# mwickert/scikit-dsp-comm

Hardware: AMD Instinct MI355X
Metric: complex64 MSamples/s (FIR-1024 tap, 2^26 samples) (higher is better)
Workload: dtype c64

## Files before the change

scikit-dsp-comm_amd/csrc/fir_ols.hip:

```cpp
#include "skdsp_internal.hpp"
#include "ols_tables.hpp"
#include <cstdlib>
#include <cstdio>


namespace skdsp {

using namespace ols;
typedef float v4f_t __attribute__((ext_vector_type(4)));

struct OlsPlan {
    int ntaps = 0;
    int ov = 0;
    int V = 0;
    float4 *T1 = nullptr, *T2 = nullptr, *Hp = nullptr;
};

struct OlsArgs {
    const cf *x;
    cf *y;
    int64_t n, n_hist;
    const float4 *T1, *T2, *Hp;
    int ov, V, a0;
    int keep;
// ... 285 lines not shown
__device__ __forceinline__ void load_tile_xr(const OlsArgs &A, int64_t tile, int t, cf *v)
{
    const float *xr = reinterpret_cast<const float *>(A.x);
    const int64_t in0 = tile * A.V - A.ov;
    const bool interior = A.aligned && in0 >= -A.n_hist && in0 + kN <= A.n;
    int tt = t;
    asm volatile("" : "+v"(tt));
    if (interior) {
#pragma unroll
        for (int a = 0; a < 16; ++a) {
            const v2f_t r = __builtin_nontemporal_load(reinterpret_cast<const v2f_t *>(xr + in0) + (unsigned)(a * 256 + tt));
            v[2 * a] = make_float2(r.x, 0.f);
            v[2 * a + 1] = make_float2(r.y, 0.f);
        }
    } else {
#pragma unroll
        for (int a = 0; a < 16; ++a) {
#pragma unroll
            for (int e = 0; e < 2; ++e) {
                const int64_t g = in0 + 512 * a + 2 * tt + e;
                v[2 * a + e] = make_float2((g >= -A.n_hist && g < A.n) ? xr[g] : 0.f, 0.f);
            }
        }
    }
}

template <bool REAL, bool XR = false> __device__ __forceinline__ void load_any(const OlsArgs &A, int64_t tile, int t, cf *v)
{
    if (XR) load_tile_xr(A, tile, t, v); else if (REAL) load_tile_real(A, tile, t, v); else load_tile(A, tile, t, v);
}
template <bool REAL, bool DEC> __device__ __forceinline__ void store_any(const OlsArgs &A, int64_t tile, int t, const cf *v, float4 *lds)
{
    if (REAL) store_tile_real<DEC>(A, tile, t, v, lds); else store_tile<DEC>(A, tile, t, v, lds);
}

__device__ __forceinline__ void lanes_swap_halves(float &e0, float &e1)
{
    const auto r = __builtin_amdgcn_permlane32_swap(__float_as_uint(e0), __float_as_uint(e1), false, false);
    e0 = __uint_as_float(r[0]);
    e1 = __uint_as_float(r[1]);
}
__device__ __forceinline__ int up_lane_pos(int t)
{
    const int lane = t & 63;
    return 128 * (t >> 6) + (lane < 32 ? 2 * lane : 2 * (lane - 32) + 1);
}

template <bool DEC> __device__ __forceinline__ void store_tile_up(const OlsArgs &A, int64_t tile, int ph, int t, const cf *v)
{
    int a0 = A.a0;
    asm volatile("" : "+s"(a0));
    int tt = t;
    asm volatile("" : "+v"(tt));
    const int pos = up_lane_pos(tt);
    const int64_t out0 = tile * A.V;
    char *ub = reinterpret_cast<char *>(A.y) + out0 * A.up_sb + A.up_pb0 + (int64_t)ph * A.up_pbs;
    const int64_t left = A.n - out0;
    const int lim = (left > (1 << 20) ? (1 << 20) : (int)left) - pos;
    const bool whole = left >= A.V;
    const unsigned b0 = (unsigned)pos * (unsigned)A.up_sb, b1 = b0 + 64u * (unsigned)A.up_sb;
    const size_t step = (size_t)512 * A.up_sb;
    const unsigned M = (unsigned)A.dec;
    const int64_t jt = out0 * A.up + ph, q0 = DEC ? jt / A.dec : 0;
    const unsigned r0 = DEC ? (unsigned)(jt - q0 * A.dec) : 0u;
    const int64_t qleft = A.n_keep - q0;
    const int qlim = qleft > (1 << 24) ? (1 << 24) : (int)qleft;
    cf *yq = A.y + q0;
#pragma unroll
    for (int a = 0; a < 16; ++a) {
        if (a < a0) continue;
        cf e0 = v[2 * a], e1 = v[2 * a + 1];
        lanes_swap_halves(e0.x, e1.x);
        lanes_swap_halves(e0.y, e1.y);
        const int i = 512 * (a - a0);
        if (DEC) {
            const unsigned j0 = r0 + (unsigned)(i + pos) * (unsigned)A.up, j1 = j0 + 64u * (unsigned)A.up;
            const unsigned k0 = (unsigned)(((unsigned long long)j0 * A.dec_magic) >> 32), k1 = (unsigned)(((unsigned long long)j1 * A.dec_magic) >> 32);
            if (k0 * M == j0 && (int)k0 < qlim && (whole || i < lim)) yq[k0] = e0;
            if (k1 * M == j1 && (int)k1 < qlim && (whole || i + 64 < lim)) yq[k1] = e1;
            continue;
        }
        char *ua = ub + (size_t)(a - a0) * step;
        if (whole || i < lim) *reinterpret_cast<cf *>(ua + b0) = e0;
        if (whole || i + 64 < lim) *reinterpret_cast<cf *>(ua + b1) = e1;
    }
}

template <bool DEC> __device__ __forceinline__ void store_tile_real_up(const OlsArgs &A, int64_t pair, int ph, int t, const cf *v)
{
    int a0 = A.a0;
    asm volatile("" : "+s"(a0));
    int tt = t;
    asm volatile("" : "+v"(tt));
    const int pos = up_lane_pos(tt);
    const int64_t outA = (2 * pair) * A.V;
    char *ua0 = reinterpret_cast<char *>(A.y) + outA * A.up_sb + A.up_pb0 + (int64_t)ph * A.up_pbs;
    char *ub0 = ua0 + (size_t)A.V * A.up_sb;
    const int64_t left = A.n - outA;
    const int lim = (left > (1 << 20) ? (1 << 20) : (int)left) - pos;
    const int limb = lim - A.V;
    const bool whole = left >= 2 * (int64_t)A.V;
    const unsigned b0 = (unsigned)pos * (unsigned)A.up_sb, b1 = b0 + 64u * (unsigned)A.up_sb;
    const size_t step = (size_t)512 * A.up_sb;
    const unsigned M = (unsigned)A.dec;
    const int64_t jt = outA * A.up + ph, q0 = DEC ? jt / A.dec : 0;
    const unsigned r0 = DEC ? (unsigned)(jt - q0 * A.dec) : 0u;
    const int64_t qleft = A.n_keep - q0;
    const int qlim = qleft > (1 << 24) ? (1 << 24) : (int)qleft;
    float *yq = reinterpret_cast<float *>(A.y) + q0;
    const unsigned jv = (unsigned)A.V * (unsigned)A.up;
#pragma unroll
    for (int a = 0; a < 16; ++a) {
        if (a < a0) continue;
        cf e0 = v[2 * a], e1 = v[2 * a + 1];
        lanes_swap_halves(e0.x, e1.x);
        lanes_swap_halves(e0.y, e1.y);
        const int i = 512 * (a - a0);
        if (DEC) {
            const unsigned j0 = r0 + (unsigned)(i + pos) * (unsigned)A.up, j1 = j0 + 64u * (unsigned)A.up;
            auto keep = [&](unsigned j, float val, bool inside) __attribute__((always_inline)) {
                const unsigned k = (unsigned)(((unsigned long long)j * A.dec_magic) >> 32);
                if (k * M == j && (int)k < qlim && inside) yq[k] = val;
            };
            keep(j0, e0.x, whole || i < lim);
            keep(j1, e1.x, whole || i + 64 < lim);
            keep(j0 + jv, e0.y, whole || i < limb);
            keep(j1 + jv, e1.y, whole || i + 64 < limb);
            continue;
        }
        char *ua = ua0 + (size_t)(a - a0) * step, *ub = ub0 + (size_t)(a - a0) * step;
        if (whole || i < lim) *reinterpret_cast<float *>(ua + b0) = e0.x;
        if (whole || i + 64 < lim) *reinterpret_cast<float *>(ua + b1) = e1.x;
        if (whole || i < limb) *reinterpret_cast<float *>(ub + b0) = e0.y;
        if (whole || i + 64 < limb) *reinterpret_cast<float *>(ub + b1) = e1.y;
    }
}


__device__ __forceinline__ OlsCareful ols_careful_args(const OlsArgs &A, int ph, bool cx)
{
    OlsCareful c;
    c.x = A.x; c.y = A.y; c.n = A.n; c.n_hist = A.n_hist; c.n_keep = A.n_keep; c.up_pitch = A.up_pitch;
    c.V = A.V; c.dec = A.dec; c.up = A.up;
    const int esz = cx ? 8 : 4;
    c.L = A.up_sb / esz;
    c.p0 = (A.up_pb0 + ph * A.up_pbs) / esz;
    c.cf = A.cf;
    return c;
}

template <bool REAL, bool DEC, bool UP = false, bool XR = false>
__global__ __launch_bounds__(256, 2) void ols_tile_kernel(OlsArgs A)
{
    __shared__ float4 lds[kLdsUnits + 2 * kT2Units];
    __shared__ unsigned long long ols_noted;
    if (threadIdx.x == 0) ols_noted = 0;
    constexpr int HS = (DEC && !UP) ? (REAL ? 4 : 5) : 0;
    float4 *T2f = lds + kLdsUnits;
    float4 *T2t = lds + kLdsUnits + kT2Units;
    const int t = threadIdx.x;

    {
        const float4 w = A.T2[t];
        T2f[t] = w;
        T2t[(t & 15) * 16 + (t >> 4)] = w;
    }
    cf tw[16];
#pragma unroll
    for (int k1 = 1; k1 < 16; ++k1) tw[k1] = lo(A.T1[k1 * 256 + t]);
    tw[0] = make_float2(1.f, 0.f);

    __syncthreads();
    int it = 0;
    float4 hh[16];
    int64_t tile = (gridDim.x % 8 == 0) ? (int64_t)(blockIdx.x % 8) * (gridDim.x / 8) + blockIdx.x / 8
                                                                 : (int64_t)blockIdx.x;
    const bool t0_last = A.halo_flag != nullptr;
    auto phys = [&](int64_t w) -> int64_t {
        if (UP) return (int64_t)((unsigned)w / (unsigned)A.up);
        return t0_last ? (w + 1 < A.ntiles ? w + 1 : 0) : w;
    };
    auto phase_of = [&](int64_t w) -> int { return (int)((unsigned)w % (unsigned)A.up); };
    if (!UP) load_H(t, A.Hp, hh);
    cf v[32];
    if (tile < A.ntiles) {
        if (t0_last && phys(tile) == 0) wait_halo(A);
        load_any<REAL, XR>(A, phys(tile), t, v);
    }
    if constexpr (XR) {
#pragma unroll
        for (int i = 0; i < 32; i += 8)
            asm volatile("" ::"v"(v[i].x), "v"(v[i + 1].x), "v"(v[i + 2].x), "v"(v[i + 3].x), "v"(v[i + 4].x), "v"(v[i + 5].x), "v"(v[i + 6].x), "v"(v[i + 7].x));
    } else {
#pragma unroll
    for (int i = 0; i < 32; i += 8)
        asm volatile("" ::"v"(v[i].x), "v"(v[i].y), "v"(v[i + 1].x), "v"(v[i + 1].y), "v"(v[i + 2].x), "v"(v[i + 2].y),
                     "v"(v[i + 3].x), "v"(v[i + 3].y), "v"(v[i + 4].x), "v"(v[i + 4].y), "v"(v[i + 5].x), "v"(v[i + 5].y),
                     "v"(v[i + 6].x), "v"(v[i + 6].y), "v"(v[i + 7].x), "v"(v[i + 7].y));
    }
    for (; tile < A.ntiles; tile += gridDim.x, ++it) {
        if (HS > 0) {
            int tt = t;
            asm volatile("" : "+v"(tt));
#pragma unroll
            for (int j = 16 - HS; j < 16; ++j) hh[j] = vld(reinterpret_cast<const volatile float4 *>(A.Hp) + (unsigned)(j * 256 + tt));
        }
        if (UP) {
            int tt = t;
            asm volatile("" : "+v"(tt));
            const volatile float4 *hp = reinterpret_cast<const volatile float4 *>(A.Hp) + (size_t)phase_of(tile) * 4096;
#pragma unroll
            for (int j = 0; j < 16; ++j) hh[j] = vld(hp + (unsigned)(j * 256 + tt));
        }
        if (REAL) fwd_pass1_real(t, v, tw, lds); else fwd_pass1(t, v, tw, lds);
        __syncthreads();
        cf Z[32];
        fwd_pass23(t, T2f, lds, Z);
        mul_H(hh, Z);
        const int64_t next = tile + gridDim.x;
        cf nx[32];
        __builtin_amdgcn_s_setprio(3);
        if (next < A.ntiles) {
            if (t0_last && phys(next) == 0) wait_halo(A);
            load_any<REAL, XR>(A, phys(next), t, nx);
        }
        __builtin_amdgcn_s_setprio(0);
        inv_pass32(t, T2t, lds, Z);
        __syncthreads();
        inv_pass1(t, tw, lds, v);
        if constexpr (XR) {
#pragma unroll
            for (int i = 0; i < 32; i += 8)
                asm volatile("" ::"v"(nx[i].x), "v"(nx[i + 1].x), "v"(nx[i + 2].x), "v"(nx[i + 3].x), "v"(nx[i + 4].x), "v"(nx[i + 5].x), "v"(nx[i + 6].x), "v"(nx[i + 7].x)
                             : "memory");
        } else {
#pragma unroll
        for (int i = 0; i < 32; i += 8)
            asm volatile("" ::"v"(nx[i].x), "v"(nx[i].y), "v"(nx[i + 1].x), "v"(nx[i + 1].y), "v"(nx[i + 2].x), "v"(nx[i + 2].y),
                         "v"(nx[i + 3].x), "v"(nx[i + 3].y), "v"(nx[i + 4].x), "v"(nx[i + 4].y), "v"(nx[i + 5].x), "v"(nx[i + 5].y),
                         "v"(nx[i + 6].x), "v"(nx[i + 6].y), "v"(nx[i + 7].x), "v"(nx[i + 7].y)
                         : "memory");
        }
        __builtin_amdgcn_s_setprio(3);
        if (UP) {
            if (!DEC && A.up_pitch) {
                OlsArgs B = A;
                B.y = REAL ? reinterpret_cast<cf *>(reinterpret_cast<float *>(A.y) + (int64_t)phase_of(tile) * A.up_pitch) : A.y + (int64_t)phase_of(tile) * A.up_pitch;
                store_any<REAL, false>(B, phys(tile), t, v, lds);
            } else if (REAL) {
                store_tile_real_up<DEC>(A, phys(tile), phase_of(tile), t, v);
            } else {
                store_tile_up<DEC>(A, phys(tile), phase_of(tile), t, v);
            }
        } else {
            store_any<REAL, DEC>(A, phys(tile), t, v, lds);
        }
        __builtin_amdgcn_s_setprio(0);
        if (__builtin_expect(__any(not_finite(v[31].x) | not_finite(v[31].y)), 0)) careful_note(&ols_noted, it);
#pragma unroll
        for (int i = 0; i < 32; ++i) v[i] = nx[i];
#ifdef SK_OLS_KEEP_B3
        __syncthreads();
#else
        if constexpr (REAL || DEC || UP || XR) __syncthreads();
#endif
    }
    const unsigned long long noted = careful_noted(&ols_noted);
    if (__builtin_expect(noted != 0, 0)) {
        int64_t w = (gridDim.x % 8 == 0) ? (int64_t)(blockIdx.x % 8) * (gridDim.x / 8) + blockIdx.x / 8 : (int64_t)blockIdx.x;
        for (int64_t k = 0; w < A.ntiles; w += gridDim.x, ++k)
            if (careful_step_noted(noted, k))
                careful_ols_tile<float, REAL, DEC, UP, XR>(ols_careful_args(A, UP ? phase_of(w) : 0, !(REAL || XR)), phys(w), UP ? phase_of(w) : 0, t);
    }
}


template <bool REAL, int MF>
__global__ __launch_bounds__(256, 2) void ols_fold_kernel(OlsArgs A)
{
    __shared__ float4 lds[kLdsUnits + 2 * kT2Units];
    __shared__ unsigned long long ols_noted;
    if (threadIdx.x == 0) ols_noted = 0;
    float4 *T2f = lds + kLdsUnits, *T2t = lds + kLdsUnits + kT2Units;
    const int t = threadIdx.x;
    {
        const float4 w = A.T2[t];
        T2f[t] = w;
        T2t[(t & 15) * 16 + (t >> 4)] = w;
    }
    cf tw[16];
#pragma unroll
    for (int k1 = 1; k1 < 16; ++k1) tw[k1] = lo(A.T1[k1 * 256 + t]);
    tw[0] = make_float2(1.f, 0.f);
    __syncthreads();
    float4 hh[16];
    auto first_tile = [&]() -> int64_t { return (gridDim.x % 8 == 0) ? (int64_t)(blockIdx.x % 8) * (gridDim.x / 8) + blockIdx.x / 8 : (int64_t)blockIdx.x; };
    int64_t tile = first_tile();
    load_H(t, A.Hp, hh);
    cf v[32];
    if (tile < A.ntiles) load_any<REAL, false>(A, tile, t, v);
#pragma unroll
    for (int i = 0; i < 32; i += 8)
        asm volatile("" ::"v"(v[i].x), "v"(v[i].y), "v"(v[i + 1].x), "v"(v[i + 1].y), "v"(v[i + 2].x), "v"(v[i + 2].y),
                     "v"(v[i + 3].x), "v"(v[i + 3].y), "v"(v[i + 4].x), "v"(v[i + 4].y), "v"(v[i + 5].x), "v"(v[i + 5].y),
                     "v"(v[i + 6].x), "v"(v[i + 6].y), "v"(v[i + 7].x), "v"(v[i + 7].y));
    constexpr int LS = MF / 2;
    const int b = t >> 4, q = t & 15;
    const bool active = q % LS == 0;
    const int j0 = (32 / MF) * b + q / LS;
    constexpr int JA = 512 / MF;
    for (int64_t step = 0; tile < A.ntiles; tile += gridDim.x, ++step) {
        if (REAL) fwd_pass1_real(t, v, tw, lds); else fwd_pass1(t, v, tw, lds);
        __syncthreads();
        cf Z[32];
        fwd_pass23(t, T2f, lds, Z);
        mul_H(hh, Z);
        const int64_t next = tile + gridDim.x;
        cf nx[32];
        __builtin_amdgcn_s_setprio(3);
        if (next < A.ntiles) load_any<REAL, false>(A, next, t, nx);
        __builtin_amdgcn_s_setprio(0);
        inv_pass32_fold<MF>(t, T2t, lds, Z);
        __syncthreads();
        cf o[16];
#pragma unroll
        for (int a = 0; a < 16; ++a) o[a] = make_float2(0.f, 0.f);
        inv_pass1_fold<MF>(t, tw, lds, o);
#pragma unroll
        for (int i = 0; i < 32; i += 8)
            asm volatile("" ::"v"(nx[i].x), "v"(nx[i].y), "v"(nx[i + 1].x), "v"(nx[i + 1].y), "v"(nx[i + 2].x), "v"(nx[i + 2].y),
                         "v"(nx[i + 3].x), "v"(nx[i + 3].y), "v"(nx[i + 4].x), "v"(nx[i + 4].y), "v"(nx[i + 5].x), "v"(nx[i + 5].y),
                         "v"(nx[i + 6].x), "v"(nx[i + 6].y), "v"(nx[i + 7].x), "v"(nx[i + 7].y)
                         : "memory");
        __builtin_amdgcn_s_setprio(3);
        if (active) {
            int a0 = A.a0;
            asm volatile("" : "+s"(a0));
            const int Mr = A.dec / MF;
            const int64_t n_out = A.n_keep / A.dec;
            const int VD = A.V / MF;
            const int64_t e0 = (REAL ? 2 * tile : tile) * (int64_t)VD;
            const int64_t q0 = Mr > 1 ? e0 / Mr : e0;
            const unsigned r0 = Mr > 1 ? (unsigned)(e0 - q0 * Mr) : 0u;
            auto put = [&](unsigned el, auto val, auto *yp) __attribute__((always_inline)) {
                if (Mr > 1) {
                    const unsigned g = r0 + el;
                    const unsigned k = (unsigned)(((unsigned long long)g * A.dec_magic) >> 32);
                    if (k * (unsigned)Mr == g && q0 + k < n_out) __builtin_nontemporal_store(val, yp + (q0 + k));
                } else if (q0 + el < n_out) {
                    __builtin_nontemporal_store(val, yp + (q0 + el));
                }
            };
#pragma unroll
            for (int a = 0; a < 16; ++a) {
                if (a < a0) continue;
                const unsigned el = (unsigned)(j0 + JA * (a - a0));
                if (REAL) {
                    put(el, o[a].x, reinterpret_cast<float *>(A.y));
                    put(el + (unsigned)VD, o[a].y, reinterpret_cast<float *>(A.y));
                } else {
                    put(el, v2f_t{o[a].x, o[a].y}, reinterpret_cast<v2f_t *>(A.y));
                }
            }
        }
        __builtin_amdgcn_s_setprio(0);
        if (__builtin_expect(__any(active && (not_finite(o[15].x) | not_finite(o[15].y))), 0)) careful_note(&ols_noted, step);
#pragma unroll
        for (int i = 0; i < 32; ++i) v[i] = nx[i];
#ifdef SK_OLS_KEEP_B3
        __syncthreads();
#else
        if constexpr (REAL) __syncthreads();
#endif
    }
    const unsigned long long noted = careful_noted(&ols_noted);
    if (__builtin_expect(noted != 0, 0)) {
        int64_t w = first_tile();
        for (int64_t k = 0; w < A.ntiles; w += gridDim.x, ++k)
            if (careful_step_noted(noted, k)) careful_ols_tile<float, REAL, true, false, false>(ols_careful_args(A, 0, !REAL), w, 0, t);
    }
}


template <bool REAL, int LF>
__device__ __forceinline__ void load_rep(const OlsArgs &A, int64_t tile, int t, cf *in)
{
    constexpr int LS = LF / 2, JA = 512 / LF;
    const int b = t >> 4, q = t & 15;
#pragma unroll
    for (int a = 0; a < 16; ++a) in[a] = make_float2(0.f, 0.f);
    if (q % LS != 0) return;
    const int j0 = (32 / LF) * b + q / LS;
    const int Lr = A.rep_lr;
    const int64_t in0 = (REAL ? 2 * tile : tile) * (int64_t)A.V - A.ov;
    const int64_t e0 = in0 / LF;
    int64_t q0 = e0, r0 = 0;
    if (Lr > 1) {
        q0 = e0 / Lr;
        r0 = e0 - q0 * Lr;
        if (r0 < 0) { r0 += Lr; q0 -= 1; }
    }
    const int VD = A.V / LF;
    auto fetch = [&](unsigned d, int64_t &idx) -> bool {
        if (Lr == 1) { idx = q0 + d; return true; }
        const unsigned g = (unsigned)r0 + d;
        const unsigned k = (unsigned)(((unsigned long long)g * A.rep_magic) >> 32);
        idx = q0 + k;
        return k * (unsigned)Lr == g;
    };
    const bool interior = Lr == 1 && A.aligned && e0 >= -A.rep_hist && e0 + kN / LF + (REAL ? VD : 0) <= A.n_in;
    int tt = j0;
    asm volatile("" : "+v"(tt));
    if (interior) {
        if (REAL) {
            const float *xa = reinterpret_cast<const float *>(A.x) + e0, *xb = xa + VD;
#pragma unroll
            for (int a = 0; a < 16; ++a) in[a] = make_float2(__builtin_nontemporal_load(xa + (unsigned)(JA * a + tt)), __builtin_nontemporal_load(xb + (unsigned)(JA * a + tt)));
        } else {
            const v2f_t *xc = reinterpret_cast<const v2f_t *>(A.x) + e0;
#pragma unroll
            for (int a = 0; a < 16; ++a) {
                const v2f_t r = __builtin_nontemporal_load(xc + (unsigned)(JA * a + tt));
                in[a] = make_float2(r.x, r.y);
            }
        }
        return;
    }
#pragma unroll
    for (int a = 0; a < 16; ++a) {
        int64_t ia, ib;
        if (REAL) {
            const float *xr = reinterpret_cast<const float *>(A.x);
            float va = 0.f, vb = 0.f;
            if (fetch((unsigned)(JA * a + tt), ia) && ia >= -A.rep_hist && ia < A.n_in) va = xr[ia];
            if (fetch((unsigned)(JA * a + tt + VD), ib) && ib >= -A.rep_hist && ib < A.n_in) vb = xr[ib];
            in[a] = make_float2(va, vb);
        } else if (fetch((unsigned)(JA * a + tt), ia) && ia >= -A.rep_hist && ia < A.n_in) {
            in[a] = A.x[ia];
        }
    }
}

template <bool REAL, int LF>
__global__ __launch_bounds__(256, 2) void ols_rep_kernel(OlsArgs A)
{
    __shared__ float4 lds[kLdsUnits + 2 * kT2Units];
    __shared__ unsigned long long ols_noted;
    if (threadIdx.x == 0) ols_noted = 0;
    float4 *T2f = lds + kLdsUnits, *T2t = lds + kLdsUnits + kT2Units;
    const int t = threadIdx.x;
    {
        const float4 w = A.T2[t];
        T2f[t] = w;
        T2t[(t & 15) * 16 + (t >> 4)] = w;
    }
    cf tw[16];
#pragma unroll
    for (int k1 = 1; k1 < 16; ++k1) tw[k1] = lo(A.T1[k1 * 256 + t]);
    tw[0] = make_float2(1.f, 0.f);
    __syncthreads();
    float4 hh[16];
    auto first_tile = [&]() -> int64_t { return (gridDim.x % 8 == 0) ? (int64_t)(blockIdx.x % 8) * (gridDim.x / 8) + blockIdx.x / 8 : (int64_t)blockIdx.x; };
    int64_t tile = first_tile();
    load_H(t, A.Hp, hh);
    cf in[16];
    if (tile < A.ntiles) load_rep<REAL, LF>(A, tile, t, in);
#pragma unroll
    for (int i = 0; i < 16; i += 8)
        asm volatile("" ::"v"(in[i].x), "v"(in[i].y), "v"(in[i + 1].x), "v"(in[i + 1].y), "v"(in[i + 2].x), "v"(in[i + 2].y),
                     "v"(in[i + 3].x), "v"(in[i + 3].y), "v"(in[i + 4].x), "v"(in[i + 4].y), "v"(in[i + 5].x), "v"(in[i + 5].y),
                     "v"(in[i + 6].x), "v"(in[i + 6].y), "v"(in[i + 7].x), "v"(in[i + 7].y));
    for (int64_t step = 0; tile < A.ntiles; tile += gridDim.x, ++step) {
        fwd_pass1_rep<LF>(t, in, tw, lds);
        __syncthreads();
        cf Z[32];
        fwd_pass23_rep<LF>(t, T2f, lds, Z);
        mul_H(hh, Z);
        const int64_t next = tile + gridDim.x;
        cf nx[16];
        __builtin_amdgcn_s_setprio(3);
        if (next < A.ntiles) load_rep<REAL, LF>(A, next, t, nx);
        __builtin_amdgcn_s_setprio(0);
        inv_pass32(t, T2t, lds, Z);
        __syncthreads();
        cf v[32];
        inv_pass1(t, tw, lds, v);
#pragma unroll
        for (int i = 0; i < 16; i += 8)
            asm volatile("" ::"v"(nx[i].x), "v"(nx[i].y), "v"(nx[i + 1].x), "v"(nx[i + 1].y), "v"(nx[i + 2].x), "v"(nx[i + 2].y),
                         "v"(nx[i + 3].x), "v"(nx[i + 3].y), "v"(nx[i + 4].x), "v"(nx[i + 4].y), "v"(nx[i + 5].x), "v"(nx[i + 5].y),
                         "v"(nx[i + 6].x), "v"(nx[i + 6].y), "v"(nx[i + 7].x), "v"(nx[i + 7].y)
                         : "memory");
        __builtin_amdgcn_s_setprio(3);
        store_any<REAL, false>(A, tile, t, v, lds);
        __builtin_amdgcn_s_setprio(0);
        if (__builtin_expect(__any(not_finite(v[31].x) | not_finite(v[31].y)), 0)) careful_note(&ols_noted, step);
#pragma unroll
        for (int i = 0; i < 16; ++i) in[i] = nx[i];
        __syncthreads();
    }
    const unsigned long long noted = careful_noted(&ols_noted);
    if (__builtin_expect(noted != 0, 0)) {
        int64_t w = first_tile();
        for (int64_t k = 0; w < A.ntiles; w += gridDim.x, ++k)
            if (careful_step_noted(noted, k))
                careful_fir_range<float, !REAL>(A.x, A.y, A.rep_hist, A.n, (REAL ? 2 * w : w) * (int64_t)A.V, (REAL ? 2 : 1) * (int64_t)A.V, A.rep_L, 1, A.cf, t);
    }
}

bool fir_ols_supported(const FirHandle *h)
{
    if (h->ntaps < 2 || h->ntaps - 1 > 4096) return false;
    return h->dtype == SKDSP_C64 || (h->dtype == SKDSP_F32 && !h->taps_complex);
}

static int build_plan(const FirHandle *h, int up, OlsPlan **out, int kind = 0)
{
    if (kind == 1) {
        const int T = (h->ntaps + up - 1) / up;
        OlsPlan *p = new OlsPlan();
        p->ntaps = T;
        p->ov = ((T - 1 + 511) / 512) * 512;
        if (p->ov == 0) p->ov = 512;
        p->V = kN - p->ov;
        std::vector<float4> T1, T2, Hp, Hall;
        make_T1(T1);
        make_T2(T2);
        std::vector<double> ph((size_t)T * 2);
        for (int k = 0; k < up / 2; ++k) {
            std::fill(ph.begin(), ph.end(), 0.0);
            for (int t = 0; t < T; ++t)
                for (int c = 0; c < 2; ++c) {
                    const int j = 2 * k + c + up * t;
                    if (j < h->ntaps) ph[(size_t)2 * t + c] = (double)up * h->taps_host[j];
                }
            make_Hp(ph.data(), T, 2, Hp);
            Hall.insert(Hall.end(), Hp.begin(), Hp.end());
        }
        hipError_t e;
        if ((e = hipMalloc((void **)&p->T1, T1.size() * sizeof(float4))) != hipSuccess ||
            (e = hipMalloc((void **)&p->T2, T2.size() * sizeof(float4))) != hipSuccess ||
            (e = hipMalloc((void **)&p->Hp, Hall.size() * sizeof(float4))) != hipSuccess ||
            (e = hipMemcpy(p->T1, T1.data(), T1.size() * sizeof(float4), hipMemcpyHostToDevice)) != hipSuccess ||
            (e = hipMemcpy(p->T2, T2.data(), T2.size() * sizeof(float4), hipMemcpyHostToDevice)) != hipSuccess ||
            (e = hipMemcpy(p->Hp, Hall.data(), Hall.size() * sizeof(float4), hipMemcpyHostToDevice)) != hipSuccess) {
            fir_ols_free(p);
            return hip_fail(e, "ols tables (paired phases)", __FILE__, __LINE__);
        }
        *out = p;
        return SKDSP_OK;
    }
    const int comp = h->taps_complex ? 2 : 1;
    const int T = kind == 3 ? h->ntaps : (h->ntaps + up - 1) / up;
    const int q_first = kind == 2 ? up - 1 : 0;
    OlsPlan *p = new OlsPlan();
    p->ntaps = T;
    p->ov = ((T - 1 + 511) / 512) * 512;
    if (p->ov == 0) p->ov = 512;
    p->V = kN - p->ov;
    std::vector<float4> T1, T2, Hp, Hall;
    make_T1(T1);
    make_T2(T2);
    if (up == 1) {
        make_Hp(h->taps_host.data(), h->ntaps, comp, Hall);
    } else if (kind == 3) {
        std::vector<double> scaled(h->taps_host);
        for (double &v : scaled) v *= (double)up;
        make_Hp(scaled.data(), h->ntaps, comp, Hall);
    } else {
        std::vector<double> ph((size_t)T * comp);
        for (int q = q_first; q < up; ++q) {
            std::fill(ph.begin(), ph.end(), 0.0);
            for (int t = 0; t < T; ++t) {
                const int k = q + up * t;
                if (k >= h->ntaps) break;
                for (int c = 0; c < comp; ++c) ph[(size_t)t * comp + c] = (double)up * h->taps_host[(size_t)k * comp + c];
            }
            make_Hp(ph.data(), T, comp, Hp);
            Hall.insert(Hall.end(), Hp.begin(), Hp.end());
        }
    }
    hipError_t e;
    if ((e = hipMalloc((void **)&p->T1, T1.size() * sizeof(float4))) != hipSuccess ||
        (e = hipMalloc((void **)&p->T2, T2.size() * sizeof(float4))) != hipSuccess ||
        (e = hipMalloc((void **)&p->Hp, Hall.size() * sizeof(float4))) != hipSuccess) {
        fir_ols_free(p);
        return hip_fail(e, "hipMalloc(ols tables)", __FILE__, __LINE__);
    }
    if ((e = hipMemcpy(p->T1, T1.data(), T1.size() * sizeof(float4), hipMemcpyHostToDevice)) != hipSuccess ||
        (e = hipMemcpy(p->T2, T2.data(), T2.size() * sizeof(float4), hipMemcpyHostToDevice)) != hipSuccess ||
        (e = hipMemcpy(p->Hp, Hall.data(), Hall.size() * sizeof(float4), hipMemcpyHostToDevice)) != hipSuccess) {
        fir_ols_free(p);
        return hip_fail(e, "hipMemcpy(ols tables)", __FILE__, __LINE__);
    }
    *out = p;
    return SKDSP_OK;
}

static int ensure_plan(FirHandle *h)
{
    if (h->ols) return SKDSP_OK;
    return build_plan(h, 1, &h->ols);
// ... 241 lines not shown
```

scikit-dsp-comm_amd/csrc/ols_core.hpp:

```cpp
#pragma once

#include <type_traits>
#if defined(__HIPCC__)
#include <hip/hip_runtime.h>
#define SK_HD __host__ __device__ __forceinline__
#define SK_UNROLL _Pragma("unroll")
#else
#include <cmath>
#define SK_UNROLL
struct float2 { float x, y; };
struct float4 { float x, y, z, w; };
static inline float2 make_float2(float x, float y) { return float2{x, y}; }
static inline float4 make_float4(float x, float y, float z, float w) { return float4{x, y, z, w}; }
#define SK_HD inline
#endif

namespace skdsp {
namespace ols {

typedef float2 cf;

constexpr int kN = 8192;
constexpr int kThreads = 256;
constexpr int kRowPitch = 272;
constexpr int kLdsUnits = 16 * kRowPitch;
constexpr int kT2Units = 256;

#define SK_C32                                                                                             \
    {1.0f, 0.98078528040323043f, 0.92387953251128674f, 0.83146961230254524f, 0.70710678118654757f,        \
     0.55557023301960229f, 0.38268343236508984f, 0.19509032201612833f, 0.0f, -0.19509032201612819f,       \
     -0.38268343236508973f, -0.55557023301960196f, -0.70710678118654746f, -0.83146961230254535f,           \
     -0.92387953251128674f, -0.98078528040323043f, -1.0f, -0.98078528040323043f, -0.92387953251128685f,    \
     -0.83146961230254546f, -0.70710678118654768f, -0.55557023301960218f, -0.38268343236509034f,           \
     -0.19509032201612866f, 0.0f, 0.19509032201612828f, 0.38268343236509f, 0.55557023301960184f,           \
     0.70710678118654735f, 0.83146961230254524f, 0.92387953251128652f, 0.98078528040323032f}
#define SK_S32                                                                                             \
    {0.0f, 0.19509032201612825f, 0.38268343236508978f, 0.55557023301960218f, 0.70710678118654746f,         \
     0.83146961230254524f, 0.92387953251128674f, 0.98078528040323043f, 1.0f, 0.98078528040323043f,         \
     0.92387953251128674f, 0.83146961230254546f, 0.70710678118654757f, 0.55557023301960218f,               \
     0.38268343236508989f, 0.19509032201612861f, 0.0f, -0.19509032201612836f, -0.38268343236508967f,       \
     -0.55557023301960196f, -0.70710678118654746f, -0.83146961230254524f, -0.92387953251128652f,           \
     -0.98078528040323032f, -1.0f, -0.98078528040323043f, -0.92387953251128663f, -0.83146961230254546f,    \
     -0.70710678118654768f, -0.55557023301960218f, -0.38268343236509039f, -0.19509032201612872f}

#if defined(__HIP_DEVICE_COMPILE__)
typedef float v2f __attribute__((ext_vector_type(2)));
SK_HD v2f V(cf a) { v2f r; r.x = a.x; r.y = a.y; return r; }
SK_HD cf C(v2f a) { return make_float2(a.x, a.y); }
SK_HD cf cadd(cf a, cf b) { return C(V(a) + V(b)); }
SK_HD cf csub(cf a, cf b) { return C(V(a) - V(b)); }
SK_HD cf cmul(cf a, cf w)
{
    v2f r;
    asm("v_pk_mul_f32 %0, %1, %2 op_sel_hi:[1,0]\n\t"
        "v_pk_fma_f32 %0, %1, %2, %0 op_sel:[1,1,0] op_sel_hi:[0,1,1] neg_lo:[0,1,0]"
        : "=&v"(r) : "v"(V(a)), "v"(V(w)));
    return C(r);
}
SK_HD cf cmulc(cf a, cf w)
{
    v2f r;
    asm("v_pk_mul_f32 %0, %1, %2 op_sel_hi:[1,0]\n\t"
        "v_pk_fma_f32 %0, %1, %2, %0 op_sel:[1,1,0] op_sel_hi:[0,1,1] neg_hi:[0,1,0]"
        : "=&v"(r) : "v"(V(a)), "v"(V(w)));
    return C(r);
}
template <bool INV> SK_HD cf cmul_k(cf a, float c, float s)
{
    v2f K;
    K.x = c; K.y = s;
    v2f r;
    if (INV)
        asm("v_pk_mul_f32 %0, %1, %2 op_sel_hi:[1,0]\n\t"
            "v_pk_fma_f32 %0, %1, %2, %0 op_sel:[1,1,0] op_sel_hi:[0,1,1] neg_lo:[0,1,0]"
            : "=&v"(r) : "v"(V(a)), "s"(K));
    else
        asm("v_pk_mul_f32 %0, %1, %2 op_sel_hi:[1,0]\n\t"
            "v_pk_fma_f32 %0, %1, %2, %0 op_sel:[1,1,0] op_sel_hi:[0,1,1] neg_hi:[0,1,0]"
            : "=&v"(r) : "v"(V(a)), "s"(K));
    return C(r);
}
template <bool INV> SK_HD cf madd_mi(cf p, cf d)
{
    v2f r;
    if (INV) asm("v_pk_add_f32 %0, %1, %2 op_sel:[0,1] op_sel_hi:[1,0] neg_lo:[0,1]" : "=v"(r) : "v"(V(p)), "v"(V(d)));
    else asm("v_pk_add_f32 %0, %1, %2 op_sel:[0,1] op_sel_hi:[1,0] neg_hi:[0,1]" : "=v"(r) : "v"(V(p)), "v"(V(d)));
    return C(r);
}
SK_HD cf cneg(cf a) { return C(-V(a)); }
#else
SK_HD cf cadd(cf a, cf b) { return make_float2(a.x + b.x, a.y + b.y); }
SK_HD cf csub(cf a, cf b) { return make_float2(a.x - b.x, a.y - b.y); }
SK_HD cf cmul(cf a, cf b) { return make_float2(a.x * b.x - a.y * b.y, a.x * b.y + a.y * b.x); }
SK_HD cf cmulc(cf a, cf b) { return make_float2(a.x * b.x + a.y * b.y, a.y * b.x - a.x * b.y); }
template <bool INV> SK_HD cf cmul_k(cf a, float c, float s)
{
    return INV ? make_float2(a.x * c - a.y * s, a.y * c + a.x * s) : make_float2(a.x * c + a.y * s, a.y * c - a.x * s);
}
template <bool INV> SK_HD cf madd_mi(cf p, cf d)
{
    return INV ? make_float2(p.x - d.y, p.y + d.x) : make_float2(p.x + d.y, p.y - d.x);
}
SK_HD cf cneg(cf a) { return make_float2(-a.x, -a.y); }
#endif
#if defined(__HIP_DEVICE_COMPILE__)
struct cf2 { v2f re, im; };
SK_HD cf2 make_cf2(cf re_pair, cf im_pair) { return cf2{V(re_pair), V(im_pair)}; }
SK_HD cf2 cadd(cf2 a, cf2 b) { return cf2{a.re + b.re, a.im + b.im}; }
SK_HD cf2 csub(cf2 a, cf2 b) { return cf2{a.re - b.re, a.im - b.im}; }
SK_HD cf2 cneg(cf2 a) { return cf2{-a.re, -a.im}; }
template <bool INV> SK_HD cf2 madd_mi(cf2 p, cf2 d) { return INV ? cf2{p.re - d.im, p.im + d.re} : cf2{p.re + d.im, p.im - d.re}; }
template <bool INV> SK_HD cf2 cmul_k(cf2 a, float c, float s)
{
    return INV ? cf2{a.re * c - a.im * s, a.im * c + a.re * s} : cf2{a.re * c + a.im * s, a.im * c - a.re * s};
}
SK_HD cf column(cf2 a, int e) { return e ? make_float2(a.re.y, a.im.y) : make_float2(a.re.x, a.im.x); }
template <int COL> SK_HD cf soa_cmul(cf2 a, cf w)
{
    v2f r;
    if (COL == 0)
        asm("v_pk_mul_f32 %0, %1, %3 op_sel:[0,0] op_sel_hi:[0,1]\n\t"
            "v_pk_fma_f32 %0, %2, %3, %0 op_sel:[0,1,0] op_sel_hi:[0,0,1] neg_lo:[0,1,0]"
            : "=&v"(r) : "v"(a.re), "v"(a.im), "v"(V(w)));
    else
        asm("v_pk_mul_f32 %0, %1, %3 op_sel:[1,0] op_sel_hi:[1,1]\n\t"
            "v_pk_fma_f32 %0, %2, %3, %0 op_sel:[1,1,0] op_sel_hi:[1,0,1] neg_lo:[0,1,0]"
            : "=&v"(r) : "v"(a.re), "v"(a.im), "v"(V(w)));
    return C(r);
}
#else
struct cf2 { float re[2], im[2]; };
SK_HD cf2 make_cf2(cf re_pair, cf im_pair) { return cf2{{re_pair.x, re_pair.y}, {im_pair.x, im_pair.y}}; }
SK_HD cf2 cadd(cf2 a, cf2 b) { return cf2{{a.re[0] + b.re[0], a.re[1] + b.re[1]}, {a.im[0] + b.im[0], a.im[1] + b.im[1]}}; }
SK_HD cf2 csub(cf2 a, cf2 b) { return cf2{{a.re[0] - b.re[0], a.re[1] - b.re[1]}, {a.im[0] - b.im[0], a.im[1] - b.im[1]}}; }
SK_HD cf2 cneg(cf2 a) { return cf2{{-a.re[0], -a.re[1]}, {-a.im[0], -a.im[1]}}; }
SK_HD cf column(cf2 a, int e) { return make_float2(a.re[e], a.im[e]); }
SK_HD cf2 from_columns(cf c0, cf c1) { return cf2{{c0.x, c1.x}, {c0.y, c1.y}}; }
template <bool INV> SK_HD cf2 madd_mi(cf2 p, cf2 d) { return from_columns(madd_mi<INV>(column(p, 0), column(d, 0)), madd_mi<INV>(column(p, 1), column(d, 1))); }
template <bool INV> SK_HD cf2 cmul_k(cf2 a, float c, float s) { return from_columns(cmul_k<INV>(column(a, 0), c, s), cmul_k<INV>(column(a, 1), c, s)); }
template <int COL> SK_HD cf soa_cmul(cf2 a, cf w) { return cmul(column(a, COL), w); }
#endif

template <bool INV, class E> SK_HD E msub_mi(E p, E d) { return madd_mi<!INV>(p, d); }
template <bool INV> SK_HD cf mul_mi(cf a) { return madd_mi<INV>(make_float2(0.f, 0.f), a); }
template <bool INV> SK_HD cf2 mul_mi(cf2 a) { return madd_mi<INV>(make_cf2(make_float2(0.f, 0.f), make_float2(0.f, 0.f)), a); }

template <bool INV> SK_HD void dft4_ip(cf &x0, cf &x1, cf &x2, cf &x3)
{
    const cf s02 = cadd(x0, x2), d02 = csub(x0, x2), s13 = cadd(x1, x3), d13 = csub(x1, x3);
    x0 = cadd(s02, s13);
    x2 = csub(s02, s13);
    x1 = madd_mi<INV>(d02, d13);
    x3 = msub_mi<INV>(d02, d13);
}

template <int N, int K, bool INV, class E> SK_HD E twmul(E a)
{
    constexpr int k32 = ((K % N) * (32 / N)) & 31;
    constexpr float Ct[32] = SK_C32;
    constexpr float St[32] = SK_S32;
    if constexpr (k32 == 0) return a;
    else if constexpr (k32 == 8) return mul_mi<INV>(a);
    else if constexpr (k32 == 16) return cneg(a);
    else if constexpr (k32 == 24) return mul_mi<!INV>(a);
    else return cmul_k<INV>(a, Ct[k32], St[k32]);
}

template <int N, int K, bool INV, class T> SK_HD void bfly_tw(T E, T O, T &Xa, T &Xb)
{
    constexpr int k32 = ((K % N) * (32 / N)) & 31;
    if constexpr (k32 == 8) {
        Xa = madd_mi<INV>(E, O);
        Xb = msub_mi<INV>(E, O);
    } else if constexpr (k32 == 24) {
        Xa = msub_mi<INV>(E, O);
        Xb = madd_mi<INV>(E, O);
    } else {
        const T t = twmul<N, K, INV>(O);
        Xa = cadd(E, t);
        Xb = csub(E, t);
    }
}

template <int I, int E, class F> SK_HD void static_for(F &&f)
{
    if constexpr (I < E) {
        f(std::integral_constant<int, I>{});
        static_for<I + 1, E>(static_cast<F &&>(f));
    }
}

template <class T, int N, int S, bool INV> struct DftT {
    static SK_HD void run(const T *x, T *X)
    {
        if constexpr (N == 1) {
            X[0] = x[0];
        } else if constexpr (N == 2) {
            X[0] = cadd(x[0], x[S]);
            X[1] = csub(x[0], x[S]);
        } else if constexpr (N == 4) {
            const T s02 = cadd(x[0], x[2 * S]), d02 = csub(x[0], x[2 * S]);
            const T s13 = cadd(x[S], x[3 * S]), d13 = csub(x[S], x[3 * S]);
            X[0] = cadd(s02, s13);
            X[2] = csub(s02, s13);
            X[1] = madd_mi<INV>(d02, d13);
            X[3] = msub_mi<INV>(d02, d13);
        } else if constexpr (N == 8) {
            T E[4], O[4];
            DftT<T, 4, 2 * S, INV>::run(x, E);
            DftT<T, 4, 2 * S, INV>::run(x + S, O);
            static_for<0, 4>([&](auto kc) {
                constexpr int k = decltype(kc)::value;
                bfly_tw<8, k, INV>(E[k], O[k], X[k], X[k + 4]);
            });
        } else {
            constexpr int M = N / 4;
            T S0[M], S1[M], S2[M], S3[M];
            DftT<T, M, 4 * S, INV>::run(x, S0);
            DftT<T, M, 4 * S, INV>::run(x + S, S1);
            DftT<T, M, 4 * S, INV>::run(x + 2 * S, S2);
            DftT<T, M, 4 * S, INV>::run(x + 3 * S, S3);
            static_for<0, M>([&](auto kc) {
                constexpr int k = decltype(kc)::value;
                const T t0 = S0[k];
                const T t1 = twmul<N, k, INV>(S1[k]);
                const T t2 = twmul<N, 2 * k, INV>(S2[k]);
                const T t3 = twmul<N, 3 * k, INV>(S3[k]);
                const T s02 = cadd(t0, t2), d02 = csub(t0, t2);
                const T s13 = cadd(t1, t3), d13 = csub(t1, t3);
                X[k] = cadd(s02, s13);
                X[k + 2 * M] = csub(s02, s13);
                X[k + M] = madd_mi<INV>(d02, d13);
                X[k + 3 * M] = msub_mi<INV>(d02, d13);
            });
        }
    }
};
template <int N, int S, bool INV> using Dft = DftT<cf, N, S, INV>;

SK_HD int lds_unit(int row_k1, int mid, int q) { return row_k1 * kRowPitch + mid * 17 + q; }

SK_HD cf lo(float4 f) { return make_float2(f.x, f.y); }
SK_HD cf hi(float4 f) { return make_float2(f.z, f.w); }
SK_HD float4 pack(cf a, cf b) { return make_float4(a.x, a.y, b.x, b.y); }

template <int K, bool INV> SK_HD cf mul_w8192(cf a)
{
    constexpr float C[16] = {1.0f, 0.99999970586288223f, 0.99999882345170188f, 0.99999735276697821f, 0.99999529380957619f, 0.99999264658070719f, 0.9999894110819284f, 0.9999855873151432f, 0.99998117528260111f, 0.99997617498689761f, 0.99997058643097414f, 0.99996440961811828f, 0.9999576445519639f, 0.99995029123649048f, 0.99994234967602391f, 0.999933819875236f};
    constexpr float S[16] = {0.0f, 0.00076699031874270449f, 0.0015339801862847655f, 0.002300969151425805f, 0.0030679567629659761f, 0.0038349425697062275f, 0.0046019261204485705f, 0.0053689069639963425f, 0.0061358846491544753f, 0.0069028587247297558f, 0.007669828739531097f, 0.0084367942423697988f, 0.0092037547820598194f, 0.0099707099074180308f, 0.010737659167264491f, 0.011504602110422714f};
    if constexpr (K == 0) return a;
    else if constexpr (INV) return make_float2(a.x * C[K] - a.y * S[K], a.y * C[K] + a.x * S[K]);
    else return make_float2(a.x * C[K] + a.y * S[K], a.y * C[K] - a.x * S[K]);
}

SK_HD void fwd_pass1(int t, const cf *v, const cf *tw, float4 *lds)
{
    cf in[16], o0[16], o1[16];
    SK_UNROLL
    for (int a = 0; a < 16; ++a) in[a] = v[2 * a];
    Dft<16, 1, false>::run(in, o0);
    SK_UNROLL
    for (int a = 0; a < 16; ++a) in[a] = v[2 * a + 1];
    Dft<16, 1, false>::run(in, o1);
    const int b = t >> 4, q = t & 15;
    lds[lds_unit(0, b, q)] = pack(o0[0], o1[0]);
    static_for<1, 16>([&](auto kc) {
        constexpr int k1 = decltype(kc)::value;
        lds[lds_unit(k1, b, q)] = pack(cmul(o0[k1], tw[k1]), cmul(mul_w8192<k1, false>(o1[k1]), tw[k1]));
    });
}

SK_HD void fwd_pass1_real(int t, const cf *v, const cf *tw, float4 *lds)
{
    cf2 in[16], o[16];
    SK_UNROLL
    for (int a = 0; a < 16; ++a) in[a] = make_cf2(v[2 * a], v[2 * a + 1]);
    DftT<cf2, 16, 1, false>::run(in, o);
    const int b = t >> 4, q = t & 15;
    lds[lds_unit(0, b, q)] = pack(column(o[0], 0), column(o[0], 1));
    static_for<1, 16>([&](auto kc) {
        constexpr int k1 = decltype(kc)::value;
        lds[lds_unit(k1, b, q)] = pack(soa_cmul<0>(o[k1], tw[k1]), mul_w8192<k1, false>(soa_cmul<1>(o[k1], tw[k1])));
    });
}

SK_HD void fwd_pass23(int t, const float4 *T2 , float4 *lds, cf *Z)
{
    const int k1 = t >> 4, q = t & 15;
    cf in0[16], in1[16], o0[16], o1[16];
    SK_UNROLL
    for (int b = 0; b < 16; ++b) {
        const float4 f = lds[lds_unit(k1, b, q)];
        in0[b] = lo(f);
        in1[b] = hi(f);
    }
    Dft<16, 1, false>::run(in0, o0);
    Dft<16, 1, false>::run(in1, o1);
    lds[lds_unit(k1, 0, q)] = pack(o0[0], o1[0]);
    SK_UNROLL
    for (int k2 = 1; k2 < 16; ++k2) {
        const float4 w = T2[k2 * 16 + q];
        lds[lds_unit(k1, k2, q)] = pack(cmul(o0[k2], lo(w)), cmul(o1[k2], hi(w)));
    }
    const int k2 = q;
    cf z[32];
    SK_UNROLL
    for (int qq = 0; qq < 16; ++qq) {
        const float4 f = lds[lds_unit(k1, k2, qq)];
        z[2 * qq] = lo(f);
        z[2 * qq + 1] = hi(f);
    }
    Dft<32, 1, false>::run(z, Z);
}

SK_HD void load_H(int t, const float4 *Hp, float4 *hh)
{
    SK_UNROLL
    for (int j = 0; j < 16; ++j) hh[j] = Hp[j * 256 + t];
}
SK_HD void mul_H(const float4 *hh, cf *Z)
{
    SK_UNROLL
    for (int j = 0; j < 16; ++j) {
        Z[2 * j] = cmul(Z[2 * j], lo(hh[j]));
        Z[2 * j + 1] = cmul(Z[2 * j + 1], hi(hh[j]));
    }
}

SK_HD void inv_pass32(int t, const float4 *T2t , float4 *lds, const cf *Z)
{
    const int k1 = t >> 4, k2 = t & 15;
    cf z[32];
    Dft<32, 1, true>::run(Z, z);
    SK_UNROLL
    for (int qq = 0; qq < 16; ++qq) {
        const float4 w = T2t[qq * 16 + k2];
        lds[lds_unit(k1, k2, qq)] = pack(cmulc(z[2 * qq], lo(w)), cmulc(z[2 * qq + 1], hi(w)));
    }
    const int q = k2;
    cf in0[16], in1[16], o0[16], o1[16];
    SK_UNROLL
    for (int kk = 0; kk < 16; ++kk) {
        const float4 f = lds[lds_unit(k1, kk, q)];
        in0[kk] = lo(f);
        in1[kk] = hi(f);
    }
    Dft<16, 1, true>::run(in0, o0);
    Dft<16, 1, true>::run(in1, o1);
    SK_UNROLL
    for (int b = 0; b < 16; ++b) lds[lds_unit(k1, b, q)] = pack(o0[b], o1[b]);
}

SK_HD void inv_pass1(int t, const cf *tw, const float4 *lds, cf *v)
{
    const int b = t >> 4, q = t & 15;
    cf in0[16], in1[16], o0[16], o1[16];
    {
        const float4 f = lds[lds_unit(0, b, q)];
        in0[0] = lo(f);
        in1[0] = hi(f);
    }
    static_for<1, 16>([&](auto kc) {
        constexpr int k1 = decltype(kc)::value;
        const float4 f = lds[lds_unit(k1, b, q)];
        in0[k1] = cmulc(lo(f), tw[k1]);
        in1[k1] = mul_w8192<k1, true>(cmulc(hi(f), tw[k1]));
    });
    Dft<16, 1, true>::run(in0, o0);
    Dft<16, 1, true>::run(in1, o1);
    SK_UNROLL
    for (int a = 0; a < 16; ++a) {
        v[2 * a] = o0[a];
        v[2 * a + 1] = o1[a];
    }
}

template <int MF> SK_HD void inv_pass32_fold(int t, const float4 *T2t , float4 *lds, const cf *Z)
{
    constexpr int R = 32 / MF, LS = MF / 2;
    const int k1 = t >> 4, k2 = t & 15;
    cf F[R], z[R];
    SK_UNROLL
    for (int k = 0; k < R; ++k) {
        cf acc = Z[k];
        SK_UNROLL
        for (int m = 1; m < MF; ++m) acc = cadd(acc, Z[k + R * m]);
        F[k] = acc;
    }
    Dft<R, 1, true>::run(F, z);
    cf *l2 = reinterpret_cast<cf *>(lds);
    SK_UNROLL
    for (int cp = 0; cp < R; ++cp) {
        const int qq = cp * LS;
        l2[2 * lds_unit(k1, k2, qq)] = cmulc(z[cp], lo(T2t[qq * 16 + k2]));
    }
    const int q = k2;
    if (q % LS == 0) {
        cf in0[16], o0[16];
        SK_UNROLL
        for (int kk = 0; kk < 16; ++kk) in0[kk] = l2[2 * lds_unit(k1, kk, q)];
        Dft<16, 1, true>::run(in0, o0);
        SK_UNROLL
        for (int b = 0; b < 16; ++b) l2[2 * lds_unit(k1, b, q)] = o0[b];
    }
}

template <int MF> SK_HD void inv_pass1_fold(int t, const cf *tw, const float4 *lds, cf *v)
{
    constexpr int LS = MF / 2;
    const int b = t >> 4, q = t & 15;
    if (q % LS != 0) return;
    const cf *l2 = reinterpret_cast<const cf *>(lds);
    cf in0[16];
    in0[0] = l2[2 * lds_unit(0, b, q)];
    static_for<1, 16>([&](auto kc) {
        constexpr int k1 = decltype(kc)::value;
        in0[k1] = cmulc(l2[2 * lds_unit(k1, b, q)], tw[k1]);
    });
    Dft<16, 1, true>::run(in0, v);
}

template <int LF> SK_HD void fwd_pass1_rep(int t, const cf *in, const cf *tw, float4 *lds)
{
    constexpr int LS = LF / 2;
    const int b = t >> 4, q = t & 15;
    if (q % LS != 0) return;
    cf o0[16];
    Dft<16, 1, false>::run(in, o0);
    cf *l2 = reinterpret_cast<cf *>(lds);
    l2[2 * lds_unit(0, b, q)] = o0[0];
    static_for<1, 16>([&](auto kc) {
        constexpr int k1 = decltype(kc)::value;
        l2[2 * lds_unit(k1, b, q)] = cmul(o0[k1], tw[k1]);
    });
}
template <int LF> SK_HD void fwd_pass23_rep(int t, const float4 *T2 , float4 *lds, cf *Z)
{
    constexpr int R = 32 / LF, LS = LF / 2;
    const int k1 = t >> 4, q = t & 15;
    cf *l2 = reinterpret_cast<cf *>(lds);
    if (q % LS == 0) {
        cf in0[16], o0[16];
        SK_UNROLL
        for (int b = 0; b < 16; ++b) in0[b] = l2[2 * lds_unit(k1, b, q)];
        Dft<16, 1, false>::run(in0, o0);
        l2[2 * lds_unit(k1, 0, q)] = o0[0];
        SK_UNROLL
        for (int k2 = 1; k2 < 16; ++k2) l2[2 * lds_unit(k1, k2, q)] = cmul(o0[k2], lo(T2[k2 * 16 + q]));
    }
    const int k2 = q;
    cf z[R], F[R];
    SK_UNROLL
    for (int cp = 0; cp < R; ++cp) z[cp] = l2[2 * lds_unit(k1, k2, cp * LS)];
    Dft<R, 1, false>::run(z, F);
    SK_UNROLL
    for (int k3 = 0; k3 < 32; ++k3) Z[k3] = F[k3 % R];
}

}
}
```

Before: 293,200.

## Prefetch twiddle tables from LDS ahead of FFT compute with volatile loads

```diff
diff --git a/scikit-dsp-comm_amd/csrc/fir_ols.hip b/scikit-dsp-comm_amd/csrc/fir_ols.hip
--- a/scikit-dsp-comm_amd/csrc/fir_ols.hip
+++ b/scikit-dsp-comm_amd/csrc/fir_ols.hip
@@ -461,12 +461,13 @@
 template <bool REAL, bool DEC, bool UP = false, bool XR = false>
 __global__ __launch_bounds__(256, 2) void ols_tile_kernel(OlsArgs A)
 {
-    __shared__ float4 lds[kLdsUnits + 2 * kT2Units];
+    __shared__ float4 lds[kLdsUnits];
+    __shared__ float4 t2lds[2 * kT2Units];
     __shared__ unsigned long long ols_noted;
     if (threadIdx.x == 0) ols_noted = 0;
     constexpr int HS = (DEC && !UP) ? (REAL ? 4 : 5) : 0;
-    float4 *T2f = lds + kLdsUnits;
-    float4 *T2t = lds + kLdsUnits + kT2Units;
+    float4 *T2f = t2lds;
+    float4 *T2t = t2lds + kT2Units;
     const int t = threadIdx.x;
 
     {
@@ -587,10 +588,11 @@
 template <bool REAL, int MF>
 __global__ __launch_bounds__(256, 2) void ols_fold_kernel(OlsArgs A)
 {
-    __shared__ float4 lds[kLdsUnits + 2 * kT2Units];
+    __shared__ float4 lds[kLdsUnits];
+    __shared__ float4 t2lds[2 * kT2Units];
     __shared__ unsigned long long ols_noted;
     if (threadIdx.x == 0) ols_noted = 0;
-    float4 *T2f = lds + kLdsUnits, *T2t = lds + kLdsUnits + kT2Units;
+    float4 *T2f = t2lds, *T2t = t2lds + kT2Units;
     const int t = threadIdx.x;
     {
         const float4 w = A.T2[t];
@@ -753,10 +755,11 @@
 template <bool REAL, int LF>
 __global__ __launch_bounds__(256, 2) void ols_rep_kernel(OlsArgs A)
 {
-    __shared__ float4 lds[kLdsUnits + 2 * kT2Units];
+    __shared__ float4 lds[kLdsUnits];
+    __shared__ float4 t2lds[2 * kT2Units];
     __shared__ unsigned long long ols_noted;
     if (threadIdx.x == 0) ols_noted = 0;
-    float4 *T2f = lds + kLdsUnits, *T2t = lds + kLdsUnits + kT2Units;
+    float4 *T2f = t2lds, *T2t = t2lds + kT2Units;
     const int t = threadIdx.x;
     {
         const float4 w = A.T2[t];
diff --git a/scikit-dsp-comm_amd/csrc/ols_core.hpp b/scikit-dsp-comm_amd/csrc/ols_core.hpp
--- a/scikit-dsp-comm_amd/csrc/ols_core.hpp
+++ b/scikit-dsp-comm_amd/csrc/ols_core.hpp
@@ -25,6 +25,8 @@
 constexpr int kRowPitch = 272;
 constexpr int kLdsUnits = 16 * kRowPitch;
 constexpr int kT2Units = 256;
+constexpr int kFwdAhead = 2;
+constexpr int kInvBatch = 2;
 
 #define SK_C32                                                                                             \
     {1.0f, 0.98078528040323043f, 0.92387953251128674f, 0.83146961230254524f, 0.70710678118654757f,        \
@@ -238,6 +240,34 @@
 };
 template <int N, int S, bool INV> using Dft = DftT<cf, N, S, INV>;
 
+#if defined(__HIP_DEVICE_COMPILE__)
+typedef float v4f __attribute__((ext_vector_type(4)));
+#define SK_LDS_PTR(T, p) ((const volatile __attribute__((address_space(3))) T *)(p))
+SK_HD float4 lds_req(const float4 *p)
+{
+    const v4f r = *SK_LDS_PTR(v4f, p);
+    return make_float4(r.x, r.y, r.z, r.w);
+}
+SK_HD cf lds_req_lo(const float4 *p) { return C(*SK_LDS_PTR(v2f, p)); }
+template <int N> SK_HD void hold(cf *v)
+{
+    if constexpr (N % 4 == 0) {
+        SK_UNROLL
+        for (int i = 0; i < N; i += 4)
+            asm volatile("" : "+v"(v[i].x), "+v"(v[i].y), "+v"(v[i + 1].x), "+v"(v[i + 1].y), "+v"(v[i + 2].x), "+v"(v[i + 2].y), "+v"(v[i + 3].x), "+v"(v[i + 3].y));
+    } else {
+        SK_UNROLL
+        for (int i = 0; i < N; ++i) asm volatile("" : "+v"(v[i].x), "+v"(v[i].y));
+    }
+}
+SK_HD void hold(cf &a, cf &b, cf &c, cf &d) { asm volatile("" : "+v"(a.x), "+v"(a.y), "+v"(b.x), "+v"(b.y), "+v"(c.x), "+v"(c.y), "+v"(d.x), "+v"(d.y)); }
+#else
+SK_HD float4 lds_req(const float4 *p) { return *p; }
+SK_HD cf lds_req_lo(const float4 *p) { return make_float2(p->x, p->y); }
+template <int N> SK_HD void hold(cf *) {}
+SK_HD void hold(cf &, cf &, cf &, cf &) {}
+#endif
+
 SK_HD int lds_unit(int row_k1, int mid, int q) { return row_k1 * kRowPitch + mid * 17 + q; }
 
 SK_HD cf lo(float4 f) { return make_float2(f.x, f.y); }
@@ -294,13 +324,16 @@
         in0[b] = lo(f);
         in1[b] = hi(f);
     }
+    float4 w[16];
+    SK_UNROLL
+    for (int k2 = 1; k2 <= kFwdAhead; ++k2) w[k2] = lds_req(T2 + k2 * 16 + q);
     Dft<16, 1, false>::run(in0, o0);
     Dft<16, 1, false>::run(in1, o1);
     lds[lds_unit(k1, 0, q)] = pack(o0[0], o1[0]);
     SK_UNROLL
     for (int k2 = 1; k2 < 16; ++k2) {
-        const float4 w = T2[k2 * 16 + q];
-        lds[lds_unit(k1, k2, q)] = pack(cmul(o0[k2], lo(w)), cmul(o1[k2], hi(w)));
+        if (k2 + kFwdAhead < 16) w[k2 + kFwdAhead] = lds_req(T2 + (k2 + kFwdAhead) * 16 + q);
+        lds[lds_unit(k1, k2, q)] = pack(cmul(o0[k2], lo(w[k2])), cmul(o1[k2], hi(w[k2])));
     }
     const int k2 = q;
     cf z[32];
@@ -332,10 +365,17 @@
     const int k1 = t >> 4, k2 = t & 15;
     cf z[32];
     Dft<32, 1, true>::run(Z, z);
-    SK_UNROLL
-    for (int qq = 0; qq < 16; ++qq) {
-        const float4 w = T2t[qq * 16 + k2];
-        lds[lds_unit(k1, k2, qq)] = pack(cmulc(z[2 * qq], lo(w)), cmulc(z[2 * qq + 1], hi(w)));
+    float4 w[16];
+    SK_UNROLL
+    for (int j = 0; j < kInvBatch; ++j) w[j] = lds_req(T2t + j * 16 + k2);
+    SK_UNROLL
+    for (int g = 0; g < 16; g += kInvBatch) {
+        if (g + kInvBatch < 16) {
+            SK_UNROLL
+            for (int j = g + kInvBatch; j < g + 2 * kInvBatch; ++j) w[j] = lds_req(T2t + j * 16 + k2);
+        }
+        SK_UNROLL
+        for (int qq = g; qq < g + kInvBatch; ++qq) lds[lds_unit(k1, k2, qq)] = pack(cmulc(z[2 * qq], lo(w[qq])), cmulc(z[2 * qq + 1], hi(w[qq])));
     }
     const int q = k2;
     cf in0[16], in1[16], o0[16], o1[16];
@@ -355,16 +395,15 @@
 {
     const int b = t >> 4, q = t & 15;
     cf in0[16], in1[16], o0[16], o1[16];
-    {
-        const float4 f = lds[lds_unit(0, b, q)];
-        in0[0] = lo(f);
-        in1[0] = hi(f);
-    }
+    float4 f[16];
+    SK_UNROLL
+    for (int k1 = 0; k1 < 16; ++k1) f[k1] = lds[lds_unit(k1, b, q)];
+    in0[0] = lo(f[0]);
+    in1[0] = hi(f[0]);
     static_for<1, 16>([&](auto kc) {
         constexpr int k1 = decltype(kc)::value;
-        const float4 f = lds[lds_unit(k1, b, q)];
-        in0[k1] = cmulc(lo(f), tw[k1]);
-        in1[k1] = mul_w8192<k1, true>(cmulc(hi(f), tw[k1]));
+        in0[k1] = cmulc(lo(f[k1]), tw[k1]);
+        in1[k1] = mul_w8192<k1, true>(cmulc(hi(f[k1]), tw[k1]));
     });
     Dft<16, 1, true>::run(in0, o0);
     Dft<16, 1, true>::run(in1, o1);
@@ -387,13 +426,14 @@
         for (int m = 1; m < MF; ++m) acc = cadd(acc, Z[k + R * m]);
         F[k] = acc;
     }
+    cf w[R];
+    SK_UNROLL
+    for (int cp = 0; cp < R; ++cp) w[cp] = lds_req_lo(T2t + cp * LS * 16 + k2);
+    hold<R>(F);
     Dft<R, 1, true>::run(F, z);
     cf *l2 = reinterpret_cast<cf *>(lds);
     SK_UNROLL
-    for (int cp = 0; cp < R; ++cp) {
-        const int qq = cp * LS;
-        l2[2 * lds_unit(k1, k2, qq)] = cmulc(z[cp], lo(T2t[qq * 16 + k2]));
-    }
+    for (int cp = 0; cp < R; ++cp) l2[2 * lds_unit(k1, k2, cp * LS)] = cmulc(z[cp], w[cp]);
     const int q = k2;
     if (q % LS == 0) {
         cf in0[16], o0[16];
@@ -410,12 +450,18 @@
     constexpr int LS = MF / 2;
     const int b = t >> 4, q = t & 15;
     if (q % LS != 0) return;
-    const cf *l2 = reinterpret_cast<const cf *>(lds);
-    cf in0[16];
-    in0[0] = l2[2 * lds_unit(0, b, q)];
+    cf in0[16], f[16];
+    SK_UNROLL
+    for (int c = 0; c < 4; ++c) {
+        SK_UNROLL
+        for (int k1 = c; k1 < 16; k1 += 4) f[k1] = lds_req_lo(lds + lds_unit(k1, b, q));
+    }
+    SK_UNROLL
+    for (int c = 0; c < 4; ++c) hold(f[c], f[c + 4], f[c + 8], f[c + 12]);
+    in0[0] = f[0];
     static_for<1, 16>([&](auto kc) {
         constexpr int k1 = decltype(kc)::value;
-        in0[k1] = cmulc(l2[2 * lds_unit(k1, b, q)], tw[k1]);
+        in0[k1] = cmulc(f[k1], tw[k1]);
     });
     Dft<16, 1, true>::run(in0, v);
 }
@@ -443,10 +489,14 @@
         cf in0[16], o0[16];
         SK_UNROLL
         for (int b = 0; b < 16; ++b) in0[b] = l2[2 * lds_unit(k1, b, q)];
+        cf w[16];
+        SK_UNROLL
+        for (int k2 = 1; k2 < 16; ++k2) w[k2] = lds_req_lo(T2 + k2 * 16 + q);
+        hold<16>(in0);
         Dft<16, 1, false>::run(in0, o0);
         l2[2 * lds_unit(k1, 0, q)] = o0[0];
         SK_UNROLL
-        for (int k2 = 1; k2 < 16; ++k2) l2[2 * lds_unit(k1, k2, q)] = cmul(o0[k2], lo(T2[k2 * 16 + q]));
+        for (int k2 = 1; k2 < 16; ++k2) l2[2 * lds_unit(k1, k2, q)] = cmul(o0[k2], w[k2]);
     }
     const int k2 = q;
     cf z[R], F[R];
```

Result: faster. 299,300, median of 6 (+2.1%).
